# Bowen951209/raytracing-book

Measured on AMD Instinct MI355X. Metric: Msamples/sec (W×H×spp/s) on Book-2 final scene @1080p, 1/2/4/8 GPUs, higher is better.
Workload: dtype f32

## Files before the change

### include/rt/rt_debug.h

```cpp
#ifndef RT_DEBUG_H
#define RT_DEBUG_H

#include <stddef.h>

#ifdef __cplusplus
extern "C" {
#endif

int rt_debug_eval_builtin(int device, int fn, const float* x, const float* y, float* out, int n);

int rt_debug_threaded_bvh(const void* nodes, size_t nbytes, void* out, size_t out_cap, int* n_out);

int rt_debug_fast_tables(const void* bvh, size_t nbytes, const void* quads, size_t qbytes, const void* boxes,
                         size_t bbytes, int n_spheres, void* nodes_out, size_t nodes_cap, int* n_per_octant,
                         unsigned int* info_out, size_t info_cap, int* slots_out, int* n_slots);

int rt_debug_link_nodes(const void* bvh, size_t nbytes, void* out, size_t out_cap, int* n_f4);
int rt_debug_link_nodes_vbox(const void* bvh, size_t nbytes, const float* vbox, int n_box, void* out,
                             size_t out_cap, int* n_f4, int* n_nodes);
int rt_debug_collapse_links(const void* bvh, size_t nbytes, const float cam[28], int width, int height, int rebuild,
                            void* out, size_t out_cap, int* n_f4, unsigned char* drop, size_t drop_cap,
                            int* n_dropped);

int rt_debug_perlin_pack(const float* texels, int w, int h, void* out, size_t out_cap);
// ... 16 lines not shown

int rt_debug_device_count(void);

int rt_debug_ab_build(void);

enum {
    RT_OPTION_BOX_PRETEST = 1,
    RT_OPTION_FASTDIV = 2,
    RT_OPTION_SPH_LDS = 3,
    RT_OPTION_BIG_WG = 4,
    RT_OPTION_CHUNK_TARGET = 5,
    RT_OPTION_STAGED_CHUNK_TARGET = 6,
    RT_OPTION_STAGE_TILES = 7,
    RT_OPTION_SM_BATCH = 8,
    RT_OPTION_SM_FRAC = 9,
    RT_OPTION_WALK_FRAC = 10,
    RT_OPTION_WATCHDOG_MS = 11,
    RT_OPTION_CHUNK_WAIT_MS = 12,
    RT_OPTION_LDS_NODE_CAP = 13,
    RT_OPTION_COMPACT_BOXES = 14,
    RT_OPTION_SPINE = 15,
    RT_OPTION_TL_LEAF_LDS = 16,
    RT_OPTION_PERLIN_PACKED = 17,
    RT_OPTION_SPARSE_STAGE = 18,
    RT_OPTION_SPHERE_PAIRS = 19,
    RT_OPTION_LEAF_PREFETCH = 20,
    RT_OPTION_TL_SMALL_LDS = 21,
    RT_OPTION_SHADE_LDS = 22,
    RT_OPTION_BOX_VNODES = 23,
    RT_OPTION_ZERO_DIR_END = 24,
    RT_OPTION_COLLAPSE = 25,
    RT_OPTION_REBUILD = 26,
    RT_OPTION_TAIL_CHUNKS = 27,
    RT_OPTION_KERNEL_VARIANT = 100,
    RT_OPTION_DEBUG_FLAGS = 101
};
int rt_debug_set_option(struct rt_ctx* ctx, int option, int value);
int rt_debug_get_option(struct rt_ctx* ctx, int option, int* value);

int rt_debug_last_launch(struct rt_ctx* ctx, int* out, int n);

int rt_debug_walk_bvh(struct rt_ctx* ctx, void* out, size_t out_cap, size_t* nbytes);

int rt_debug_build_sah_bvh(const void* spheres, size_t sph_bytes, const void* quads, size_t quad_bytes,
                           const void* media, size_t med_bytes, const void* boxes, size_t box_bytes,
                           const void* bvh, size_t bvh_bytes, int order, const float eye[3],
                           float prim_cost, void* out, size_t out_cap, size_t* nbytes);

#ifdef __cplusplus
}
#endif

#endif
```

### raytracing-book_amd/csrc/rt_capi.hip

```cpp
#include <hip/hip_runtime.h>

#include <algorithm>
#include <chrono>
#include <climits>
#include <cmath>
#include <cstdio>
#include <cstdlib>
#include <cstring>
#include <functional>
#include <map>
#include <string>
#include <thread>
#include <vector>

#include <dlfcn.h>
#include <rccl/rccl.h>

#include "rt/rt.h"
#include "rt/rt_debug.h"
#include "rt/rt_types.h"
#include "rt_device.h"
#include "bvh_sah.h"

namespace {
// ... 88 lines not shown
    std::vector<float4> inner2;
    std::vector<uint2> leaves2;
    int depth = 0;
};

}

struct rt_ctx {
    std::vector<Device> devs;
    std::string err;
    std::vector<uint8_t> host_buf[6];
    bool uploaded[6] = {false, false, false, false, false, false};
    int tex_format[8] = {0}, tex_w[8] = {0}, tex_h[8] = {0};
    rt_camera_ubo cam{};
    bool have_cam = false;
    int max_depth = 5;
    float background[3] = {0, 0, 0};
    float sqrt_spp = 1.0f, recip_sqrt_spp = 1.0f;
    int width = 0, height = 0;
    int proc_rank = 0, proc_world = 1, stripe_rows = 16;
    int n_dnodes = 0;
    std::vector<rt_dnode> dnodes;
    int bvh_mode = RT_BVH_REFERENCE;
    int n_link_nodes = 0;
    std::vector<uint8_t> sah_bvh;
    std::vector<rt_dnode> walk_dn;
    std::vector<float4> walk_links;
    int n_walk_nodes = 0;
    bool walk_v = false;
    float walk_v_margin = -1.0f;
    bool walk_stale = true;
    std::vector<float4> boxc_host;
    bool box_vnodes = true;
    bool zero_dir_end = true;
    bool collapse = true;
    int rebuild = 2;
    bool walk_r = false;
    int walk_rmode = 0;
    std::vector<rt_dnode> rb_dn;
    int rb_mode = -1;
    bool walk_c = false;
    rt_camera_ubo walk_cam{};
    int walk_w = 0, walk_h = 0;
    int n_dropped = 0;
    int n_rebuilt = 0;
    int n_vnodes = 0;
    FastTables fast;
    std::vector<float4> links;
    int fast_gen = 0;
    bool spec_ok = false;
    int debug_flags = 0;
    bool uv_always = false;
    bool boxes_canon = false;
    bool fd_ok[6] = {true, true, true, true, true, true};
    bool fd_cam = true;
    bool boxes_cond = false;
    float scene_extent = -1.0f;
    bool validated = false;
    uint64_t last_ns = 0;
    int variant = 0;
    int variant_no_stats = -1;
    std::vector<int64_t> inj_hits;
    int64_t inj_walks = 0;
    int chunk_target = 16;
    int staged_chunk_target = 48;
    int tail_chunks = -1;
// ... 1710 lines not shown
    a.chunk_wait_ticks = c->chunk_wait_ticks;
    int32_t lc = 0;
    if (c->host_buf[RT_BIND_LIGHTS].size() >= 4) std::memcpy(&lc, c->host_buf[RT_BIND_LIGHTS].data(), 4);
    a.lights_count = lc;
    a.uv_always = c->uv_always;
    a.boxes_canon = c->boxes_canon ? 1 : 0;
    if (c->scene_extent < 0.0f) c->scene_extent = scene_extent(c);
    a.box_margin = (c->boxes_cond && c->box_pretest && c->scene_extent <= 0x1p60f)
                       ? std::max(c->scene_extent, 1.0f) * 0x1p-13f
                       : 0.0f;
    a.fastdiv = (c->fastdiv && c->fd_cam && c->fd_ok[RT_BIND_SPHERES] && c->fd_ok[RT_BIND_QUADS] &&
                 c->fd_ok[RT_BIND_BOXES])
                    ? 1
                    : 0;
    a.variant = c->variant;
    a.zero_dir_end = c->zero_dir_end ? 1 : 0;
    a.sm_batch = c->sm_batch;
    a.walk_frac = c->walk_frac ? c->walk_frac : walk_frac_for(c->n_link_nodes);
    const FastTables& F = c->fast;
    a.fast_ok = F.ok ? 1 : 0;
    a.n_f2inner = (int)(F.inner2.size() / 4);
    a.n_f2leaves = (int)F.leaves2.size();
    a.f2depth = F.depth;
    std::memcpy(a.finfo_base, F.base, sizeof(a.finfo_base));
    a.fm_n = F.fm_n;
    std::memcpy(a.fm_medium, F.fm_medium, sizeof(a.fm_medium));
    std::memcpy(a.fm_leaf, F.fm_leaf, sizeof(a.fm_leaf));
    std::memcpy(a.fm_track, F.fm_track, sizeof(a.fm_track));
    std::memcpy(a.fm_flags, F.fm_flags, sizeof(a.fm_flags));
    a.fl_n = F.fl_n;
    std::memcpy(a.fl_medium, F.fl_medium, sizeof(a.fl_medium));
    std::memcpy(a.fl_rank, F.fl_rank, sizeof(a.fl_rank));
    a.debug_flags = c->debug_flags;
    {
        const size_t nb = c->host_buf[RT_BIND_BOXES].size() / sizeof(rt_box);
        const bool all_cmp = c->compact_boxes && nb > 0 && c->n_boxc_ok == (int)nb;
        const bool use_v = c->box_vnodes && all_cmp && a.box_margin > 0.0f && (c->variant == 0 || c->variant == 39) &&
                           c->boxc_host.size() == nb * RT_BOXC_F4;
        const bool use_c = c->collapse && (c->variant == 0 || c->variant == 39) && c->have_cam;
        const bool cam_moved = use_c && (std::memcmp(&c->walk_cam, &c->cam, sizeof(rt_camera_ubo)) != 0 ||
                                         c->walk_w != c->width || c->walk_h != c->height);
        const bool use_r = c->rebuild > 0 && (c->variant == 0 || c->variant == 39);
        if (c->walk_stale || use_v != c->walk_v || (use_v && a.box_margin != c->walk_v_margin) ||
            use_c != c->walk_c || cam_moved || use_r != c->walk_r || c->rebuild != c->walk_rmode) {
            if (c->walk_stale) c->rb_mode = -1;
            if (use_r && c->rb_mode != c->rebuild) {
                c->rb_dn = rebuild_inner(c->walk_dn, c->rebuild);
                c->rb_mode = c->rebuild;
            }
            static const std::vector<rt_dnode> none;
            const std::vector<rt_dnode>& rb = use_r ? c->rb_dn : none;
            const std::vector<rt_dnode>& wdn = rb.empty() ? c->walk_dn : rb;
            std::vector<uint8_t> drop;
            if (use_c) {
                try {
                    if (!c->inj_hits.empty() && c->inj_hits.size() >= wdn.size()) {
                        std::vector<uint32_t> order{0u};
                        for (size_t q = 0; q < order.size() && order.size() <= wdn.size(); q++) {
                            const uint32_t k = order[q];
                            if ((wdn[k].meta & 0xF0000u) != 0 || k + 1 >= wdn.size()) continue;
                            order.push_back(k + 1);
                            order.push_back(wdn[k + 1].meta & 0xFFFFu);
                        }
                        std::vector<int64_t> H(wdn.size(), 0);
                        if (order.size() == wdn.size())
                            for (size_t q = 0; q < order.size(); q++)
// ... 931 lines not shown
        int r = d2h(c, d, tmp.data(), d.stats.ptr, sizeof(unsigned long long) * n);
        if (r) return r;
        for (int i = 0; i < n; i++) out[i] += tmp[i];
    }
    return RT_OK;
}

int rt_debug_ab_build(void) {
#ifdef RT_AB_KNOBS
    return 1;
#else
    return 0;
#endif
}

int rt_debug_set_option(rt_ctx* c, int option, int v) {
    if (!c) return RT_ERR_INVALID_ARG;
    auto bad = [&]() { return set_err(c, RT_ERR_INVALID_ARG, "option value out of range"); };
    switch (option) {
        case RT_OPTION_BOX_PRETEST: c->box_pretest = v != 0; break;
        case RT_OPTION_FASTDIV: c->fastdiv = v != 0; break;
        case RT_OPTION_SPH_LDS: c->sph_lds = v != 0; break;
        case RT_OPTION_BIG_WG: c->big_wg = v != 0; break;
        case RT_OPTION_COMPACT_BOXES: c->compact_boxes = v != 0; break;
        case RT_OPTION_SPINE: c->spine = v != 0; break;
        case RT_OPTION_TL_LEAF_LDS: c->tl_leaf_lds = v != 0; break;
        case RT_OPTION_PERLIN_PACKED: c->perlin_pk = v != 0; break;
        case RT_OPTION_SPARSE_STAGE: c->sparse_stage = v != 0; break;
        case RT_OPTION_SPHERE_PAIRS: if (v < 0 || v > 2) return bad(); c->sphere_pairs = v; break;
        case RT_OPTION_LEAF_PREFETCH: c->leaf_prefetch = v != 0; break;
        case RT_OPTION_TL_SMALL_LDS: c->tl_small_lds = v != 0; break;
        case RT_OPTION_SHADE_LDS: c->shade_lds = v != 0; break;
        case RT_OPTION_BOX_VNODES: c->box_vnodes = v != 0; break;
        case RT_OPTION_ZERO_DIR_END: c->zero_dir_end = v != 0; break;
        case RT_OPTION_COLLAPSE: c->collapse = v != 0; break;
        case RT_OPTION_REBUILD: if (v < 0 || v > 2) return bad(); c->rebuild = v; break;
        case RT_OPTION_CHUNK_TARGET: if (v < 0) return bad(); c->chunk_target = v; break;
        case RT_OPTION_STAGED_CHUNK_TARGET: if (v < 1) return bad(); c->staged_chunk_target = v; break;
        case RT_OPTION_STAGE_TILES: if (v < 0) return bad(); c->stage_tiles = v; break;
        case RT_OPTION_SM_BATCH: if (v < 1 || v > 64) return bad(); c->sm_batch = v; break;
        case RT_OPTION_SM_FRAC: if (v < 0 || v > 64) return bad(); c->sm_frac = v; break;
        case RT_OPTION_WALK_FRAC: if (v < 0 || v > 64) return bad(); c->walk_frac = v; break;
        case RT_OPTION_WATCHDOG_MS: if (v < 0) return bad(); c->watchdog_ticks = (unsigned long long)v * 100000ull; break;
        case RT_OPTION_CHUNK_WAIT_MS: if (v < 0) return bad(); c->chunk_wait_ticks = (unsigned long long)v * 100000ull; break;
        case RT_OPTION_LDS_NODE_CAP: if (v < 0) return bad(); c->lds_node_cap = v; break;
        case RT_OPTION_TAIL_CHUNKS: if (v < -1 || v > RT_MAX_FRAMES_PER_LAUNCH) return bad(); c->tail_chunks = v; break;
#ifdef RT_AB_KNOBS
        case RT_OPTION_KERNEL_VARIANT:
            if (!(v == 0 || v == 30 || v == 31 || v == 37 || v == 38 || v == 39 || v == 61 || v == 69)) return bad();
            c->variant = v;
            break;
        case RT_OPTION_DEBUG_FLAGS: c->debug_flags = v; break;
#endif
        default: return set_err(c, RT_ERR_INVALID_ARG, "unknown option (A/B options need librtamd_ab.so)");
    }
    return RT_OK;
}

int rt_debug_get_option(rt_ctx* c, int option, int* v) {
    if (!c || !v) return RT_ERR_INVALID_ARG;
    switch (option) {
        case RT_OPTION_BOX_PRETEST: *v = c->box_pretest; break;
        case RT_OPTION_FASTDIV: *v = c->fastdiv; break;
        case RT_OPTION_SPH_LDS: *v = c->sph_lds; break;
        case RT_OPTION_BIG_WG: *v = c->big_wg; break;
        case RT_OPTION_COMPACT_BOXES: *v = c->compact_boxes; break;
        case RT_OPTION_SPINE: *v = c->spine; break;
        case RT_OPTION_TL_LEAF_LDS: *v = c->tl_leaf_lds; break;
        case RT_OPTION_PERLIN_PACKED: *v = c->perlin_pk; break;
        case RT_OPTION_SPARSE_STAGE: *v = c->sparse_stage; break;
        case RT_OPTION_SPHERE_PAIRS: *v = c->sphere_pairs; break;
        case RT_OPTION_LEAF_PREFETCH: *v = c->leaf_prefetch; break;
        case RT_OPTION_TL_SMALL_LDS: *v = c->tl_small_lds; break;
        case RT_OPTION_SHADE_LDS: *v = c->shade_lds; break;
        case RT_OPTION_BOX_VNODES: *v = c->box_vnodes; break;
        case RT_OPTION_ZERO_DIR_END: *v = c->zero_dir_end; break;
        case RT_OPTION_COLLAPSE: *v = c->collapse; break;
        case RT_OPTION_REBUILD: *v = c->rebuild; break;
        case RT_OPTION_CHUNK_TARGET: *v = c->chunk_target; break;
        case RT_OPTION_STAGED_CHUNK_TARGET: *v = c->staged_chunk_target; break;
        case RT_OPTION_STAGE_TILES: *v = c->stage_tiles; break;
        case RT_OPTION_SM_BATCH: *v = c->sm_batch; break;
        case RT_OPTION_SM_FRAC: *v = c->sm_frac; break;
        case RT_OPTION_WALK_FRAC: *v = c->walk_frac; break;
        case RT_OPTION_WATCHDOG_MS: *v = (int)std::min<unsigned long long>(INT_MAX, c->watchdog_ticks / 100000ull); break;
        case RT_OPTION_CHUNK_WAIT_MS: *v = (int)std::min<unsigned long long>(INT_MAX, c->chunk_wait_ticks / 100000ull); break;
        case RT_OPTION_LDS_NODE_CAP: *v = c->lds_node_cap; break;
        case RT_OPTION_TAIL_CHUNKS: *v = c->tail_chunks; break;
#ifdef RT_AB_KNOBS
        case RT_OPTION_KERNEL_VARIANT: *v = c->variant; break;
        case RT_OPTION_DEBUG_FLAGS: *v = c->debug_flags; break;
#endif
        default: return set_err(c, RT_ERR_INVALID_ARG, "unknown option (A/B options need librtamd_ab.so)");
    }
    return RT_OK;
}

int rt_set_bvh_mode(rt_ctx* c, int mode) {
    if (!c) return RT_ERR_INVALID_ARG;
    if (mode != RT_BVH_REFERENCE && mode != RT_BVH_SAH) return set_err(c, RT_ERR_INVALID_ARG, "bad BVH mode");
    if (mode != c->bvh_mode) {
        c->bvh_mode = mode;
        c->validated = false;
    }
    return RT_OK;
}

int rt_debug_walk_bvh(rt_ctx* c, void* out, size_t out_cap, size_t* nbytes) {
// ... 53 lines not shown
```

### raytracing-book_amd/csrc/rt_device.h

```cpp
#pragma once

#include <hip/hip_runtime.h>
#include <stdint.h>

#include "rt/rt_types.h"

#define RT_MAX_FRAMES_PER_LAUNCH 512
#define RT_NODE_END 0xFFFFu
#define RT_DFACE_F4 3
#define RT_DBOX_F4 23
#define RT_BOXC_F4 3
#define RT_LDS_ACC_BYTES (512 * 16)
#define RT_LDS_DYN_BYTES (80 * 1024 - RT_LDS_ACC_BYTES)
#define RT_LDS_BIG_BYTES (160 * 1024)
#define RT_LDS_BIG_STATS_BYTES (150 * 1024)
#define RT_CENSUS_WORDS 5
#define RT_STATS_N 128
#define RT_LDS_NODE_BYTES (64 * 1024)

struct rt_dnode {
    float xmin, xmax, ymin, ymax, zmin, zmax;
    uint32_t meta;
    uint32_t prims;
};
// ... 61 lines not shown
    int perlin_slot;
    int perlin_lds;
    int perlin_packed;
    const float4* perlin_pk;
    int n_media;
    int media_sph;
    int media_lds;
    int sph_lds;
    int n_sph_lds;
    int n_box_lds;
    int sph_mat_lds;
    int box_mat_lds;
    int tex_lds;
    int tex_lds_off[8];
    int block;
    int acc_lds;
    const uint32_t* finfo;
    int fast_ok;
    int finfo_base[8];
    int fm_n;
    int fm_medium[4], fm_leaf[4], fm_track[4], fm_flags[4];
    int fl_n;
    int fl_medium[2], fl_rank[2];
    const float4* f2inner;
    const uint2* f2leaves;
    int n_f2inner, n_f2leaves, f2depth;
    const float4* lnodes;
    int n_lnode_f4;
    int lds_node_f4;
    int leaf_lds;
    int lds_end_f4;
    int box_cmp_lds;
    int box_all_cmp;
    int sph_pairs;
    int spine_len;
    uint32_t spine_start;
    float spine_lo[3], spine_hi[3];
    unsigned long long watchdog_ticks;
    unsigned long long chunk_wait_ticks;
    float rand_factors[RT_MAX_FRAMES_PER_LAUNCH];
};

enum { RT_LI_SHAPE = 0, RT_LI_BLOCK, RT_LI_FASTDIV, RT_LI_PRETEST, RT_LI_LDS, RT_LI_LDS_NODES, RT_LI_COMPACT,
       RT_LI_STAGED, RT_LI_CHUNKS, RT_LI_SPINE, RT_LI_SPARSE, RT_LI_SPAIR, RT_LI_LEAF_PF, RT_LI_SHADE_LDS, RT_LI_WALK_FRAC, RT_LI_BVH_MODE, RT_LI_VNODES, RT_LI_COLLAPSED, RT_LI_REBUILT, RT_LI_N = 20 };

#ifdef RT_AB_KNOBS
#define RT_FAST_STACK 16
enum { RT_AB_SHAPE_FAST_LDS = 0, RT_AB_SHAPE_FAST_GLOBAL, RT_AB_SHAPE_LINK_PIXEL, RT_AB_SHAPE_META_LDS,
       RT_AB_SHAPE_META_GLOBAL };
int rt_launch_render_ab(int shape, rt_kernel_args& a, const rt_kernel_args* d, size_t lds, bool stats, void* stream);
#endif
int rt_resident_waves(void);
int rt_launch_render(rt_kernel_args& a, rt_kernel_args* dargs, void* stream, int* info, void* moments = nullptr);
int rt_launch_fold_moments(const rt_kernel_args& a, void* moments, void* stream);
int rt_launch_tile_sums(const void* image, const void* moments, int width, int local_rows, void* out, void* stream);
__host__ __device__ inline void rt_gathered_row(int y, int world, int stripe_rows, int* k, int* lr) {
    const int s = y / stripe_rows;
    *k = s % world;
    *lr = (s / world) * stripe_rows + y % stripe_rows;
}
int rt_launch_deinterleave(const void* gathered, void* out, int width, int height, int world, int stripe_rows,
                           int padded_rows, void* stream);
int rt_launch_eval_builtin(int fn, const float* dx, const float* dy, float* dout, int n, void* stream);
```

### raytracing-book_amd/csrc/rt_kernel.hip

```cpp
#include "rt_kernel_common.h"

namespace {

#define RT_SM_FRESH 0
#define RT_SM_TRACE 1
#define RT_SM_HIT 2
#define RT_SM_BEGIN 4
struct UnitGeo {
    int chunk, tile, tx0, ly0, wt, ht, f0, f1;
    uint32_t total;
};
__device__ __forceinline__ UnitGeo unit_geo(const KP& P, int u, int n_tiles, int tiles_x) {
    UnitGeo g;
    g.chunk = u / n_tiles;
    g.tile = u - g.chunk * n_tiles;
    g.tx0 = (g.tile % tiles_x) * 8;
    g.ly0 = (g.tile / tiles_x) * 8;
    g.wt = min(8, P.width - g.tx0);
    g.ht = min(8, P.local_rows - g.ly0);
    const int c_main = P.n_chunks - P.tail_chunks;
    if (g.chunk < c_main) {
        g.f0 = g.chunk * P.chunk_frames;
        g.f1 = min(P.n_frames - P.tail_chunks, g.f0 + P.chunk_frames);
    } else {
// ... 219 lines not shown
        RT_ST_PART(ST_BEGIN_CYC)
        __builtin_amdgcn_s_setprio(1);
        for (;;) {
            unsigned long long th = STATS ? clock64() : 0;
            const unsigned long long tr = __ballot(status == RT_SM_TRACE);
            const int n_hit = __popcll(__ballot(status == RT_SM_HIT));
            if (STATS && tr) st_pred(st, status == RT_SM_FRESH, ST_RET_IT, ST_RET_LN);
            if (tr == 0 || n_hit >= batch || n_hit * 64 >= P.sm_frac * (n_hit + __popcll(tr))) break;
            const bool lane_exact = (inv.x == -INFINITY) || (inv.y == -INFINITY) || (inv.z == -INFINITY);
            const bool wave_exact = __ballot(status == RT_SM_TRACE && lane_exact) != 0;
            if (STATS) st_add(st, ST_RHEAD_CYC, clock64() - th);
            if (status == RT_SM_TRACE) {
                if (STATS) st_lanes(st, ST_ROUND_IT, ST_ROUND_LN);
                unsigned long long t0 = STATS ? clock64() : 0;
                if (P.walk_frac >= 64) {
                    nx = wave_exact ? link_walk<true, STATS, TL>(ns, nx, S.o, inv, 0.001f, tmax, st)
                                    : link_walk<false, STATS, TL>(ns, nx, S.o, inv, 0.001f, tmax, st);
                } else {
                    const int needw = (__popcll(__ballot(1)) * P.walk_frac + 63) >> 6;
                    nx = wave_exact ? link_walk_part<true, STATS, TL>(ns, nx, S.o, inv, 0.001f, tmax, needw, st)
                                    : link_walk_part<false, STATS, TL, (BOXC || (RT_BL_SPAIR && (OPT & RT_OPT_SPAIR) != 0)) && STD>(ns, nx, S.o, inv, 0.001f, tmax,
                                                                                    needw, st);
                }
                if (STATS) st_add(st, ST_NODE_CYC, clock64() - t0);
                if ((int)nx >= 0) {
                } else if (nx == RT_LINK_END) {
                    status = RT_SM_HIT;
                } else {
                    unsigned long long t1 = STATS ? clock64() : 0;
                    if (STATS) st_lanes(st, ST_LEAF_IT, ST_LEAF_LN);
                    uint2 lf;
                    if (gleaf) lf = ldg_u2(gleaves + (nx & 0x7FFFFFFFu));
                    else lf = leaves[nx & 0x7FFFFFFFu];
                    leaf_prims_t<STATS, FD, BOXC, (OPT & RT_OPT_SPAIR) != 0, STD>(P, lf.x << 16, lf.y, S.o, S.d, inv, a,
                                                                             S.time, 0.001f, tmax, S.rf,
                                                  fx, fy, h, has, st);
                    if (STATS) {
                        const unsigned long long t2 = clock64();
                        st_add(st, ST_LEAF_CYC, t2 - t1);
                        if (P.census) census_leaf(P, gwave, lf.x, t1, t2, __popcll(tr), st);
                    }
                    nx = lf.x >> 8;
                    if (nx == RT_LINK_NEXT_END) status = RT_SM_HIT;
                }
            }
        }
        __builtin_amdgcn_s_setprio(0);
        RT_ST_PART(ST_ROUNDS_CYC)
        if (status == RT_SM_HIT) {
            unsigned long long ts = STATS ? clock64() : 0;
            if (STATS) st_lanes(st, ST_SHADE_IT, ST_SHADE_LN);
            v3 cur3;
            h.t = tmax;
            bool done = after_trace<BOXC, STATS, STD>(P, S, h, has, fx, fy, cur3, st);
            if (!done && S.depth >= P.max_depth) {
                cur3 = mk3s(0.0f);
                done = true;
            } else if (!done && P.zero_dir_end && S.d.x == 0.0f && S.d.y == 0.0f && S.d.z == 0.0f) {
                cur3 = mul3(S.acc, mk3(P.background[0], P.background[1], P.background[2]));
                done = true;
            }
            if (done) {
                const float4 c4 = make_float4(cur3.x, cur3.y, cur3.z, 0.0f);
                if (staged) {
                    if (sparse) {
                        const bool nz = (__float_as_uint(cur3.x) | __float_as_uint(cur3.y) | __float_as_uint(cur3.z)) != 0u;
                        P.sflags[dst] = nz ? 1 : 0;
// ... 181 lines not shown
    a.leaf_pf = (a.leaf_pf && a.box_all_cmp && a.sph_lds >= 0 && a.box_cmp_lds > a.sph_lds &&
                 (a.n_media == 0 || a.media_lds >= 0)) ? 1 : 0;
    a.acc_lds = (int)(staged / 16);
    const size_t lds = staged + (pool ? 0 : RT_LDS_ACC_BYTES);
    if (info) {
        info[RT_LI_SHAPE] = (int)shape;
        info[RT_LI_BLOCK] = (shape == LINK_LDS || shape == LINK_TL) ? a.block : 512;
        info[RT_LI_FASTDIV] = a.fastdiv;
        info[RT_LI_PRETEST] = a.box_margin > 0.0f;
        info[RT_LI_LDS] = (int)lds;
        info[RT_LI_LDS_NODES] = (shape == LINK_LDS || shape == LINK_TL) ? a.lds_node_f4 / 2 : 0;
        info[RT_LI_COMPACT] = a.box_all_cmp + 2 * (a.box_cmp_lds >= 0);
        info[RT_LI_STAGED] = a.samples != nullptr;
        info[RT_LI_CHUNKS] = a.n_chunks;
        info[RT_LI_SPINE] = pool ? a.spine_len : 0;
        info[RT_LI_SPARSE] = a.samples && a.sflags ? 1 : 0;
        info[RT_LI_SPAIR] = (pool && shape == LINK_LDS && a.sph_lds >= 0 &&
                             ((a.sph_pairs && !a.box_all_cmp) || (a.sph_pairs == 2 && a.fastdiv))) ? 1 : 0;
        info[RT_LI_LEAF_PF] = (pool && (shape == LINK_LDS || shape == LINK_TL)) ? a.leaf_pf : 0;
        info[RT_LI_WALK_FRAC] = a.walk_frac;
        info[RT_LI_SHADE_LDS] = (a.sph_mat_lds >= 0) + 2 * (a.box_mat_lds >= 0) + 4 * (a.tex_lds >= 0);
    }
    if (hipMemcpyAsync(dargs, &a, sizeof(a), hipMemcpyHostToDevice, st) != hipSuccess) return -1;
    const rt_kernel_args* d = (const rt_kernel_args*)dargs;
    const int n_tiles = ((a.width + 7) / 8) * ((a.local_rows + 7) / 8);
    if (hipMemsetAsync(a.tile_counter, 0, sizeof(int), st) != hipSuccess) return -1;
    if (a.n_chunks > 1 && !a.samples &&
        hipMemsetAsync(a.tile_done, 0, sizeof(unsigned) * (size_t)n_tiles, st) != hipSuccess)
        return -1;

    constexpr int SM = RT_OPT_POOL | RT_OPT_SM | RT_OPT_STREAM;
#ifdef RT_AB_KNOBS
#define RT_KERNEL(BLOCK, OPT)                                                                            \
    (stats ? launch_persistent(render_persistent<4, true, BLOCK, OPT>, BLOCK, lds, a, d, st)                \
           : launch_persistent(render_persistent<4, false, BLOCK, OPT>, BLOCK, lds, a, d, st))
#else
#define RT_KERNEL(BLOCK, OPT) launch_persistent(render_persistent<4, false, BLOCK, OPT>, BLOCK, lds, a, d, st)
#endif
    int rc = -1;
    const bool std_cfg = a.samples && a.sflags && a.media_sph &&
                         (a.n_sph_lds == 0 || (a.sph_lds >= 0 && a.sph_mat_lds >= 0)) &&
                         (a.n_media == 0 || a.media_lds >= 0) && (a.n_box_lds == 0 || a.box_cmp_lds >= 0) &&
                         (!a.box_all_cmp || (a.leaf_pf && a.box_mat_lds >= 0)) && a.tex_lds >= 0;
#define RT_LINK4(BLOCK, OPT)                                                                                 \
    (a.fastdiv ? (a.box_all_cmp ? (std_cfg ? RT_KERNEL(BLOCK, (OPT) | RT_OPT_FD | RT_OPT_BOXC | RT_OPT_STD)            \
                                           : RT_KERNEL(BLOCK, (OPT) | RT_OPT_FD | RT_OPT_BOXC))                         \
                                : (std_cfg ? RT_KERNEL(BLOCK, (OPT) | RT_OPT_FD | RT_OPT_STD)                            \
                                           : RT_KERNEL(BLOCK, (OPT) | RT_OPT_FD)))                                      \
               : (a.box_all_cmp ? RT_KERNEL(BLOCK, (OPT) | RT_OPT_BOXC) : RT_KERNEL(BLOCK, (OPT))))
#define RT_LINK4S(BLOCK, OPT)                                                                                 \
    ((a.sph_pairs == 2 && a.box_all_cmp && a.fastdiv) ? RT_KERNEL(BLOCK, (OPT) | RT_OPT_FD | RT_OPT_BOXC | RT_OPT_SPAIR) : \
    (a.sph_pairs && !a.box_all_cmp)                                                                          \
         ? (a.fastdiv ? (std_cfg ? RT_KERNEL(BLOCK, (OPT) | RT_OPT_FD | RT_OPT_SPAIR | RT_OPT_STD)                      \
                                 : RT_KERNEL(BLOCK, (OPT) | RT_OPT_FD | RT_OPT_SPAIR))                                \
                      : RT_KERNEL(BLOCK, (OPT) | RT_OPT_SPAIR))                                                       \
         : RT_LINK4(BLOCK, OPT))
    switch (shape) {
        case LINK_LDS:
            if (!pool) {
#ifdef RT_AB_KNOBS
                rc = rt_launch_render_ab(RT_AB_SHAPE_LINK_PIXEL, a, d, lds, stats, st);
#endif
            } else if (a.block == 1024) {
                rc = RT_LINK4S(1024, SM);
            } else {
                rc = RT_LINK4S(512, SM);
            }
            break;
        case LINK_TL: rc = RT_LINK4(1024, SM | RT_OPT_TL); break;
#ifdef RT_AB_KNOBS
        case FAST_LDS: rc = rt_launch_render_ab(RT_AB_SHAPE_FAST_LDS, a, d, lds, stats, st); break;
        case FAST_GLOBAL: rc = rt_launch_render_ab(RT_AB_SHAPE_FAST_GLOBAL, a, d, lds, stats, st); break;
        case META_LDS: rc = rt_launch_render_ab(RT_AB_SHAPE_META_LDS, a, d, lds, stats, st); break;
        case META_GLOBAL: rc = rt_launch_render_ab(RT_AB_SHAPE_META_GLOBAL, a, d, lds, stats, st); break;
#endif
        default: break;
    }
#undef RT_KERNEL
// ... 28 lines not shown
```

### raytracing-book_amd/csrc/rt_kernel_common.h

```cpp
#pragma once

#include <hip/hip_runtime.h>

#include <algorithm>
#include <cstdio>
#include <cstdlib>

#include "rt/rt_glsl.h"
#include "rt_device.h"


namespace {

typedef rt_kernel_args KP;

#ifndef RT_BL_SPAIR
#define RT_BL_SPAIR 1
#endif
#define RT_OPT_POOL 1
#define RT_OPT_SM 2
#define RT_OPT_FD 4
#define RT_OPT_STREAM 8
#define RT_OPT_TL 16
#define RT_OPT_BOXC 32
#define RT_OPT_SPAIR 64
#define RT_OPT_STD 128

extern __shared__ float4 rt_dyn_lds[];

__device__ __forceinline__ v3 f3(float4 v) { return mk3(v.x, v.y, v.z); }

typedef float f4v __attribute__((ext_vector_type(4)));
typedef __attribute__((address_space(1))) const f4v g_f4v;
typedef __attribute__((address_space(1))) const float g_f;
typedef __attribute__((address_space(3))) const float lds_f;
__device__ __forceinline__ float4 ldg(const float4* p) {
    const f4v v = *(const g_f4v*)p;
    return make_float4(v.x, v.y, v.z, v.w);
}
__device__ __forceinline__ int ldg_i(const int* p) { return *(__attribute__((address_space(1))) const int*)p; }
typedef __attribute__((address_space(4))) const f4v c_f4v;
__device__ __forceinline__ float4 ldc(const float4* p) {
    const f4v v = *(const c_f4v*)p;
    return make_float4(v.x, v.y, v.z, v.w);
}
__device__ __forceinline__ int ldc_i(const int* p) { return *(__attribute__((address_space(4))) const int*)p; }
typedef unsigned u2v __attribute__((ext_vector_type(2)));
__device__ __forceinline__ uint2 ldg_u2(const uint2* p) {
    const u2v v = *(__attribute__((address_space(1))) const u2v*)p;
    return make_uint2(v.x, v.y);
}

enum {
    ST_TOTAL = 0, ST_START_CYC, ST_START_IT, ST_START_LN, ST_NODE_CYC, ST_NODE_IT, ST_NODE_LN, ST_LEAF_CYC,
    ST_LEAF_IT, ST_LEAF_LN, ST_SPH_LN, ST_QUAD_LN, ST_BOX_LN, ST_MED_LN, ST_SHADE_CYC, ST_SHADE_IT, ST_SHADE_LN,
    ST_SPH_IT, ST_QUAD_IT, ST_BOX_IT, ST_MED_IT,
    ST_FAST_TRACES, ST_FAST_EXACT, ST_FAST_WHY, ST_FAST_STEPS = ST_FAST_WHY + 9, ST_FAST_TESTS,
    ST_FAST_PRE_CYC, ST_FAST_POST_CYC, ST_FAST_EXACT_CYC,
// ... 177 lines not shown
            ti[k] = (pl.w - g_dot(n, o)) / denom;
            if (!(fabsf(denom) < 1e-8f) && (tmin <= ti[k] && ti[k] <= tmax)) cand |= 1u << k;
        }
#pragma unroll
        for (int k = 0; k < 3; k++) {
            const int i = h + k;
            if ((cand >> k) & 1u) {
                float al, be;
                if (ti[k] <= tmax && face_interior(ldg(fb + 6 + 2 * i), ldg(fb + 7 + 2 * i), o, d, ti[k], al, be, fd)) {
                    tmax = ti[k];
                    t = ti[k];
                    face = i;
                    alpha = al;
                    beta = be;
                    has = true;
                }
            }
        }
    }
    return has;
}

template <int I>
__device__ __forceinline__ void boxc_face(float mnx, float mny, float mnz, float mxx, float mxz, float DX, float DY,
                                          float DZ, float4& A, float4& B) {
    if (I == 0) { A = make_float4(mnx, mny, DX, 0.0f); B = make_float4(0.0f, DY, DX * DY, __int_as_float(0)); }
    if (I == 1) { A = make_float4(mny, mxz, 0.0f, -DZ); B = make_float4(DY, 0.0f, DZ * DY, __int_as_float(2)); }
    if (I == 2) { A = make_float4(mxx, mny, -DX, 0.0f); B = make_float4(0.0f, DY, -(DX * DY), __int_as_float(0)); }
    if (I == 3) { A = make_float4(mny, mnz, 0.0f, DZ); B = make_float4(DY, 0.0f, -(DZ * DY), __int_as_float(2)); }
    if (I == 4) { A = make_float4(mnx, mxz, DX, 0.0f); B = make_float4(0.0f, -DZ, -(DX * DZ), __int_as_float(1)); }
    if (I == 5) { A = make_float4(mnx, mnz, DX, 0.0f); B = make_float4(0.0f, DZ, DX * DZ, __int_as_float(1)); }
}
__device__ __forceinline__ bool box_test_compact(float4 c0, float4 c1, float4 c2, v3 o, v3 d, float tmin, float tmax,
                                                 float& t, int& face, float& alpha, float& beta, bool fd = false) {
    const float mnx = c0.x, mny = c0.y, mnz = c0.z, mxx = c0.w, mxy = c1.x, mxz = c1.y;
    const float sz = c1.z, sx = c1.w, sy = c2.x;
    bool has = false;
#define RT_BOXC_FACE(I, S, Q, DK, OK)                                                           \
    {                                                                                                      \
        const float s_ = (S), den = s_ * (DK);                                                             \
        float ti;                                                                                          \
        if (fd) {                                                                                          \
            ti = div_nr(s_ * (Q) - s_ * (OK), den, rcp_nr(den));                                           \
        } else {                                                                                           \
            ti = (s_ * (Q) - s_ * (OK)) / den;                                                             \
        }                                                                                                  \
        if (!(fabsf(den) < 1e-8f) && (tmin <= ti && ti <= tmax)) {                                         \
            float4 A, B;                                                                                   \
            boxc_face<I>(mnx, mny, mnz, mxx, mxz, mxx - mnx, mxy - mny, mxz - mnz, A, B);                  \
            float al, be;                                                                                  \
            if (face_interior(A, B, o, d, ti, al, be, fd)) {                                               \
                tmax = ti;                                                                                 \
                t = ti;                                                                                    \
                face = I;                                                                                  \
                alpha = al;                                                                                \
                beta = be;                                                                                 \
                has = true;                                                                                \
            }                                                                                              \
        }                                                                                                  \
    }
    RT_BOXC_FACE(0, sz, mxz, d.z, o.z)
    RT_BOXC_FACE(1, sx, mxx, d.x, o.x)
    RT_BOXC_FACE(2, -sz, mnz, d.z, o.z)
    RT_BOXC_FACE(3, -sx, mnx, d.x, o.x)
    RT_BOXC_FACE(4, sy, mxy, d.y, o.y)
    RT_BOXC_FACE(5, -sy, mny, d.y, o.y)
#undef RT_BOXC_FACE
    return has;
}

__device__ __noinline__ bool boundary_t(const KP& P, int idx, int type, v3 o, v3 d, float a, float time, float tmin,
                                           float tmax, float& t) {
    float al, be;
    int face;
    if (type == RT_MODEL_SPHERE)
        return sphere_t(reinterpret_cast<const float4*>(P.spheres + idx), time, o, d, a, tmin, tmax, t);
    if (type == RT_MODEL_QUAD) return quad_test(P.dquads + RT_DFACE_F4 * idx, o, d, tmin, tmax, t, al, be);
    if (type == RT_MODEL_BOX) return box_test(P.dboxes + RT_DBOX_F4 * idx, o, d, tmin, tmax, t, face, al, be);
    return false;
}

__device__ __forceinline__ bool sphere_bounds(float4 A, float4 B, v3 o, v3 d, float a, float time, float& t1,
                                              float& t2, bool fd = false) {
    {
        v3 center = add3(f3(A), scale3(f3(B), time));
        v3 oc = sub3(o, center);
        float half_b = g_dot(oc, d);
        float c = g_dot(oc, oc) - B.w * B.w;
        float disc = half_b * half_b - a * c;
        float sq = sqrtf(disc);
        fd = fd && __ballot(!(a >= 0x1p-60f)) == 0;
        const float ra = fd ? rcp_nr(a) : 0.0f;
        float r_lo = fd ? div_nr(-half_b - sq, a, ra) : (-half_b - sq) / a;
        float r_hi = fd ? div_nr(-half_b + sq, a, ra) : (-half_b + sq) / a;
        const bool lo_in = -RT_INFINITY < r_lo && r_lo < RT_INFINITY;
        const bool hi_in = -RT_INFINITY < r_hi && r_hi < RT_INFINITY;
        t1 = lo_in ? r_lo : r_hi;
        const float lo2 = t1 + 0.0001f;
        const bool lo_2 = lo2 < r_lo && r_lo < RT_INFINITY;
        const bool hi_2 = lo2 < r_hi && r_hi < RT_INFINITY;
// ... 89 lines not shown
    float r;
    asm("v_max_f32 %0, %1, %2" : "=v"(r) : "v"(a), "v"(b));
    return r;
}
__device__ __forceinline__ float v_min3(float a, float b, float c) {
    float r;
    asm("v_min3_f32 %0, %1, %2, %3" : "=v"(r) : "v"(a), "v"(b), "v"(c));
    return r;
}
__device__ __forceinline__ float v_max3(float a, float b, float c) {
    float r;
    asm("v_max3_f32 %0, %1, %2, %3" : "=v"(r) : "v"(a), "v"(b), "v"(c));
    return r;
}
__device__ __forceinline__ bool aabb_fast(float4 n0, float4 n1, v3 o, v3 inv, float tmin, float tmax) {
    float t0x = (n0.x - o.x) * inv.x, t1x = (n0.y - o.x) * inv.x;
    float t0y = (n0.z - o.y) * inv.y, t1y = (n0.w - o.y) * inv.y;
    float t0z = (n1.x - o.z) * inv.z, t1z = (n1.y - o.z) * inv.z;
    float lo = v_max(v_max3(tmin, v_min(t0x, t1x), v_min(t0y, t1y)), v_min(t0z, t1z));
    float hi = v_min(v_min3(tmax, v_max(t0x, t1x), v_max(t0y, t1y)), v_max(t0z, t1z));
    return !(hi <= lo);
}

typedef float f2v __attribute__((ext_vector_type(2)));
__device__ __forceinline__ bool aabb_pk(float4 n0, float4 n1, v3 o, v3 inv, float tmin, float tmax) {
    const f2v tx = (f2v{n0.x, n0.y} - f2v{o.x, o.x}) * f2v{inv.x, inv.x};
    const f2v ty = (f2v{n0.z, n0.w} - f2v{o.y, o.y}) * f2v{inv.y, inv.y};
    const f2v tz = (f2v{n1.x, n1.y} - f2v{o.z, o.z}) * f2v{inv.z, inv.z};
    float lo = v_max(v_max3(tmin, v_min(tx.x, tx.y), v_min(ty.x, ty.y)), v_min(tz.x, tz.y));
    float hi = v_min(v_min3(tmax, v_max(tx.x, tx.y), v_max(ty.x, ty.y)), v_max(tz.x, tz.y));
    return !(hi <= lo);
}

template <bool STATS, bool FD, bool BOXC = false, bool SPAIR = false, bool STD = false>
__device__ __forceinline__ void leaf_prims_t(const KP& P, uint32_t meta, uint32_t prims, v3 o, v3 d, v3 inv, float a,
                                             float time, float tmin, float& tmax, float& rf, float px, float py, Hit& h,
                                             bool& has, unsigned long long* st) {
    constexpr bool fd = FD;
    if (SPAIR && !STATS && (STD || P.sph_lds >= 0) && ((meta >> 16) & 0xFFu) == (RT_MODEL_SPHERE | (RT_MODEL_SPHERE << 4))) {
        const int i0 = (int)(prims & 0xFFFFu), i1 = (int)(prims >> 16);
        const float4* r0 = rt_dyn_lds + P.sph_lds + 2 * i0;
        const float4* r1 = rt_dyn_lds + P.sph_lds + 2 * i1;
        const float4 A0 = r0[0], B0 = r0[1], A1 = r1[0], B1 = r1[1];
        float lo0, hi0, lo1, hi1;
        const bool ok0 = sphere_roots(A0, B0, time, o, d, a, lo0, hi0, fd);
        const bool ok1 = sphere_roots(A1, B1, time, o, d, a, lo1, hi1, fd);
#pragma unroll
        for (int k = 0; k < 2; k++) {
            const bool ok = k ? ok1 : ok0;
            const int ix = k ? i1 : i0;
            float root = k ? lo1 : lo0;
            bool hit = ok && tmin < root && root < tmax;
            if (ok && !hit) {
                root = k ? hi1 : hi0;
                hit = tmin < root && root < tmax;
            }
            if (hit) {
                h.uv_kind_idx = (1 << 16) | ix;
                h.uv_a = root;
                has = true;
                tmax = root;
                h.t = root;
                h.tif = RT_MODEL_SPHERE | (ix << 16);
            }
        }
        return;
    }
// ... 44 lines not shown
                hit = sphere_t(reinterpret_cast<const float4*>(P.spheres + ix), time, o, d, a, tmin, tmax, t, fd,
                               fd ? rcp_nr(a) : 0.0f);
            }
            if (hit) { h.uv_kind_idx = (1 << 16) | ix; h.uv_a = t; }
            if (STATS) st_add(st, ST_SPH_CYC, clock64() - c0);
        } else if (ty == RT_MODEL_QUAD) {
            hit = quad_test(P.dquads + RT_DFACE_F4 * ix, o, d, tmin, tmax, t, al, be, fd);
            if (hit) { h.uv_kind_idx = 2 << 16; h.uv_a = al; h.uv_b = be; }
            if (STATS) st_add(st, ST_QUAD_CYC, clock64() - c0);
        } else if (ty == RT_MODEL_BOX) {
            float4 r0, r1, r2;
            if (pf) {
                r0 = q0;
                r1 = q1;
                r2 = q2;
            } else if (STD || P.box_cmp_lds >= 0) {
                const float4* cr = rt_dyn_lds + P.box_cmp_lds + RT_BOXC_F4 * ix;
                r0 = cr[0];
                r1 = cr[1];
                r2 = cr[2];
            } else {
                const float4* cr = P.dboxc + RT_BOXC_F4 * ix;
                r0 = ldg(cr);
                r1 = ldg(cr + 1);
                r2 = ldg(cr + 2);
            }
            bool maybe = true;
            if (P.box_margin > 0.0f && (BOXC || fin) && !pretested) {
                const float m = P.box_margin;
                maybe = aabb_pk(make_float4(r0.x - m, r0.w + m, r0.y - m, r1.x + m),
                                make_float4(r0.z - m, r1.y + m, 0.0f, 0.0f), o, inv, tmin, tmax);
            }
            if (maybe) {
                if constexpr (BOXC)
                    hit = box_test_compact(r0, r1, r2, o, d, tmin, tmax, t, face, al, be, fd);
                else
                    hit = box_test(P.dboxes + RT_DBOX_F4 * ix, o, d, tmin, tmax, t, face, al, be, fd);
            }
            if (hit) { h.uv_kind_idx = 2 << 16; h.uv_a = al; h.uv_b = be; }
            if (STATS) st_add(st, ST_BOX_CYC, clock64() - c0);
        } else if (ty == RT_MODEL_CONSTANT_MEDIUM) {
            hit = pf ? medium_test_rec<FD, STD>(P, q0, q1, q2, o, d, a, time, tmin, tmax, rf, px, py, t)
                     : medium_test<FD, STD>(P, ix, o, d, a, time, tmin, tmax, rf, px, py, t);
            if (STATS) st_add(st, ST_MED_CYC, clock64() - c0);
        }
        if (hit) {
            has = true;
            tmax = t;
            h.t = t; h.tif = ty | (face << 4) | (ix << 16);
        }
    }
}


typedef __attribute__((address_space(3))) const f4v lds_f4;
struct NodeSrc {
    const char* base;
    const char* gnodes;
    uint32_t lim;
    unsigned* hits;
};
__device__ __forceinline__ void count_node_hit(unsigned* hits, uint32_t nx, bool hit) {
    const uint32_t n0 = __builtin_amdgcn_readfirstlane(nx);
    const unsigned long long hm = __ballot(hit && nx == n0);
    if (hm && first_active_lane()) atomicAdd(&hits[n0 >> 5], (unsigned)__popcll(hm));
    if (hit && nx != n0) atomicAdd(&hits[nx >> 5], 1u);
}
template <bool STATS, bool TL>
// ... 752 lines not shown
```

### raytracing-book_amd/rtamd/render.py

```python
import ctypes
import time

import numpy as np

from . import _lib
from ._lib import RTError, c_float_p
from .scene import Scene, spp_uniforms

MASK64 = (1 << 64) - 1


def frame_rand_factors(seed, start, n):
    out = np.empty(n, dtype=np.float32)
    for k in range(n):
        z = (seed + (start + k + 1) * 0x9E3779B97F4A7C15) & MASK64
        z = ((z ^ (z >> 30)) * 0xBF58476D1CE4E5B9) & MASK64
        z = ((z ^ (z >> 27)) * 0x94D049BB133111EB) & MASK64
        z ^= z >> 31
        out[k] = np.float32(z >> 40) / np.float32(16777216.0)
    return out


def comm_unique_id(lib=None):
    L = lib or _lib.amd()
# ... 22 lines not shown
    return out.raw[:n.value]


def local_rows(height, rank, world, stripe_rows):
    n_stripes = (height + stripe_rows - 1) // stripe_rows
    return sum(min(stripe_rows, height - s * stripe_rows) for s in range(rank, n_stripes, world))


def padded_local_rows(height, world, stripe_rows):
    n_stripes = (height + stripe_rows - 1) // stripe_rows
    return ((n_stripes + world - 1) // world) * stripe_rows


def stripe_rows_of(height, rank, world, stripe_rows):
    n_stripes = (height + stripe_rows - 1) // stripe_rows
    rows = []
    for s in range(rank, n_stripes, world):
        rows.extend(range(s * stripe_rows, min(height, (s + 1) * stripe_rows)))
    return np.array(rows, dtype=np.int64)


def deinterleave(gathered, height, world, stripe_rows):
    W = gathered.shape[2]
    out = np.zeros((height, W, 4), dtype=gathered.dtype)
    for k in range(world):
        rows = stripe_rows_of(height, k, world, stripe_rows)
        out[rows] = gathered[k, :len(rows)]
    return out


OPTIONS = {"box_pretest": 1, "fastdiv": 2, "sph_lds": 3, "big_wg": 4, "chunk_target": 5,
           "staged_chunk_target": 6, "stage_tiles": 7, "sm_batch": 8, "sm_frac": 9, "walk_frac": 10,
           "watchdog_ms": 11, "chunk_wait_ms": 12, "lds_node_cap": 13, "compact_boxes": 14, "spine": 15,
           "tl_leaf_lds": 16, "perlin_packed": 17, "sparse_stage": 18, "sphere_pairs": 19, "leaf_prefetch": 20, "tl_small_lds": 21, "shade_lds": 22, "box_vnodes": 23, "zero_dir_end": 24, "collapse": 25, "rebuild": 26, "tail_chunks": 27, "kernel_variant": 100, "debug_flags": 101}
LAUNCH_FIELDS = ("shape", "block", "fastdiv", "pretest", "lds_bytes", "lds_nodes", "box_records", "staged",
                 "chunks", "spine", "sparse", "sphere_pairs", "leaf_prefetch", "shade_lds", "walk_frac", "bvh_mode",
                 "box_vnodes", "collapsed", "rebuilt")
BVH_MODES = {"reference": 0, "sah": 1}
TILE_SUM_DTYPE = np.dtype([("m2y", "<f4"), ("y", "<f4"), ("bad", "<u4"), ("pixels", "<u4")])


def noise_from_tile_sums(tiles, frames, lib=None):
    L = lib or _lib.amd()
    t = np.ascontiguousarray(tiles, dtype=TILE_SUM_DTYPE)
    s = _lib.RtNoiseStats()
    rc = L.rt_noise_from_tile_sums(t.ctypes.data_as(ctypes.POINTER(_lib.RtTileSum)), int(t.size), int(frames),
                                   ctypes.byref(s))
    if rc != 0:
        raise RTError(rc, "rt_noise_from_tile_sums: frames >= 2 required")
    return s.as_dict()
SHAPES = {0: "fast-lds", 1: "fast-global", 2: "link-lds", 3: "meta-lds", 4: "meta-global", 5: "link-two-level"}


class RenderContext:

    def __init__(self, devices=(0,), rank=0, world=1, stripe_rows=16, options=None, ab=False, lib=None):
        L = _lib.amd_at(lib) if lib else (_lib.amd_ab() if ab else _lib.amd())
        self._L = L
        devs = (ctypes.c_int * len(devices))(*devices)
        h = ctypes.c_void_p()
        rc = L.rt_create(len(devices), devs, ctypes.byref(h))
        if rc != 0:
            raise RTError(rc, L.rt_last_error(None).decode())
        self._h = h
        self.devices = tuple(devices)
        self.rank, self.world, self.stripe_rows = rank, world, stripe_rows
        if world > 1 or stripe_rows != 16:
            self._check(L.rt_set_partition(h, rank, world, stripe_rows))
        self.width = self.height = 0
        self.max_depth = 5
# ... 278 lines not shown
```

Baseline: 7416.

## Add quotient-based box face interior test deferring divisions to final hit

Adds a new compact box intersection path that tests whether a face hit lies inside the face by comparing numerators against the denominator by sign and magnitude, instead of dividing to get alpha and beta for every candidate face. The slab distances for each axis pair now share one reciprocal, and the divisions for alpha and beta run only once, for the winning face. If any lane in the wave sees tiny or degenerate numerators, the whole wave falls back to the original routine through a ballot. The path is on by default for the standard compact-box, fast-divide, non-two-level, non-stats kernel, and it adds a new kernel template instantiation.

```diff
diff --git a/include/rt/rt_debug.h b/include/rt/rt_debug.h
--- a/include/rt/rt_debug.h
+++ b/include/rt/rt_debug.h
@@ -72,6 +72,7 @@
     RT_OPTION_COLLAPSE = 25,
     RT_OPTION_REBUILD = 26,
     RT_OPTION_TAIL_CHUNKS = 27,
+    RT_OPTION_BOX_INTERIOR = 28,
     RT_OPTION_KERNEL_VARIANT = 100,
     RT_OPTION_DEBUG_FLAGS = 101
 };
diff --git a/raytracing-book_amd/csrc/rt_capi.hip b/raytracing-book_amd/csrc/rt_capi.hip
--- a/raytracing-book_amd/csrc/rt_capi.hip
+++ b/raytracing-book_amd/csrc/rt_capi.hip
@@ -144,6 +144,7 @@
     bool walk_stale = true;
     std::vector<float4> boxc_host;
     bool box_vnodes = true;
+    bool box_interior = true;
     bool zero_dir_end = true;
     bool collapse = true;
     int rebuild = 2;
@@ -1920,6 +1921,7 @@
     std::memcpy(a.fl_medium, F.fl_medium, sizeof(a.fl_medium));
     std::memcpy(a.fl_rank, F.fl_rank, sizeof(a.fl_rank));
     a.debug_flags = c->debug_flags;
+    a.box_interior = c->box_interior ? 1 : 0;
     {
         const size_t nb = c->host_buf[RT_BIND_BOXES].size() / sizeof(rt_box);
         const bool all_cmp = c->compact_boxes && nb > 0 && c->n_boxc_ok == (int)nb;
@@ -2917,6 +2919,7 @@
         case RT_OPTION_TL_SMALL_LDS: c->tl_small_lds = v != 0; break;
         case RT_OPTION_SHADE_LDS: c->shade_lds = v != 0; break;
         case RT_OPTION_BOX_VNODES: c->box_vnodes = v != 0; break;
+        case RT_OPTION_BOX_INTERIOR: c->box_interior = v != 0; break;
         case RT_OPTION_ZERO_DIR_END: c->zero_dir_end = v != 0; break;
         case RT_OPTION_COLLAPSE: c->collapse = v != 0; break;
         case RT_OPTION_REBUILD: if (v < 0 || v > 2) return bad(); c->rebuild = v; break;
@@ -2959,6 +2962,7 @@
         case RT_OPTION_TL_SMALL_LDS: *v = c->tl_small_lds; break;
         case RT_OPTION_SHADE_LDS: *v = c->shade_lds; break;
         case RT_OPTION_BOX_VNODES: *v = c->box_vnodes; break;
+        case RT_OPTION_BOX_INTERIOR: *v = c->box_interior; break;
         case RT_OPTION_ZERO_DIR_END: *v = c->zero_dir_end; break;
         case RT_OPTION_COLLAPSE: *v = c->collapse; break;
         case RT_OPTION_REBUILD: *v = c->rebuild; break;
diff --git a/raytracing-book_amd/csrc/rt_device.h b/raytracing-book_amd/csrc/rt_device.h
--- a/raytracing-book_amd/csrc/rt_device.h
+++ b/raytracing-book_amd/csrc/rt_device.h
@@ -117,6 +117,7 @@
     int lds_end_f4;
     int box_cmp_lds;
     int box_all_cmp;
+    int box_interior;
     int sph_pairs;
     int spine_len;
     uint32_t spine_start;
@@ -127,7 +128,7 @@
 };
 
 enum { RT_LI_SHAPE = 0, RT_LI_BLOCK, RT_LI_FASTDIV, RT_LI_PRETEST, RT_LI_LDS, RT_LI_LDS_NODES, RT_LI_COMPACT,
-       RT_LI_STAGED, RT_LI_CHUNKS, RT_LI_SPINE, RT_LI_SPARSE, RT_LI_SPAIR, RT_LI_LEAF_PF, RT_LI_SHADE_LDS, RT_LI_WALK_FRAC, RT_LI_BVH_MODE, RT_LI_VNODES, RT_LI_COLLAPSED, RT_LI_REBUILT, RT_LI_N = 20 };
+       RT_LI_STAGED, RT_LI_CHUNKS, RT_LI_SPINE, RT_LI_SPARSE, RT_LI_SPAIR, RT_LI_LEAF_PF, RT_LI_SHADE_LDS, RT_LI_WALK_FRAC, RT_LI_BVH_MODE, RT_LI_VNODES, RT_LI_COLLAPSED, RT_LI_REBUILT, RT_LI_BOXQ, RT_LI_N = 20 };
 
 #ifdef RT_AB_KNOBS
 #define RT_FAST_STACK 16
diff --git a/raytracing-book_amd/csrc/rt_kernel.hip b/raytracing-book_amd/csrc/rt_kernel.hip
--- a/raytracing-book_amd/csrc/rt_kernel.hip
+++ b/raytracing-book_amd/csrc/rt_kernel.hip
@@ -275,7 +275,7 @@
                     uint2 lf;
                     if (gleaf) lf = ldg_u2(gleaves + (nx & 0x7FFFFFFFu));
                     else lf = leaves[nx & 0x7FFFFFFFu];
-                    leaf_prims_t<STATS, FD, BOXC, (OPT & RT_OPT_SPAIR) != 0, STD>(P, lf.x << 16, lf.y, S.o, S.d, inv, a,
+                    leaf_prims_t<STATS, FD, BOXC, (OPT & RT_OPT_SPAIR) != 0, STD, (OPT & RT_OPT_BOXQ) != 0>(P, lf.x << 16, lf.y, S.o, S.d, inv, a,
                                                                              S.time, 0.001f, tmax, S.rf,
                                                   fx, fy, h, has, st);
                     if (STATS) {
@@ -523,7 +523,7 @@
     constexpr int SM = RT_OPT_POOL | RT_OPT_SM | RT_OPT_STREAM;
 #ifdef RT_AB_KNOBS
 #define RT_KERNEL(BLOCK, OPT)                                                                            \
-    (stats ? launch_persistent(render_persistent<4, true, BLOCK, OPT>, BLOCK, lds, a, d, st)                \
+    (stats ? launch_persistent(render_persistent<4, true, BLOCK, (OPT) & ~RT_OPT_BOXQ>, BLOCK, lds, a, d, st)  \
            : launch_persistent(render_persistent<4, false, BLOCK, OPT>, BLOCK, lds, a, d, st))
 #else
 #define RT_KERNEL(BLOCK, OPT) launch_persistent(render_persistent<4, false, BLOCK, OPT>, BLOCK, lds, a, d, st)
@@ -533,8 +533,13 @@
                          (a.n_sph_lds == 0 || (a.sph_lds >= 0 && a.sph_mat_lds >= 0)) &&
                          (a.n_media == 0 || a.media_lds >= 0) && (a.n_box_lds == 0 || a.box_cmp_lds >= 0) &&
                          (!a.box_all_cmp || (a.leaf_pf && a.box_mat_lds >= 0)) && a.tex_lds >= 0;
+    if (info)
+        info[RT_LI_BOXQ] = (pool && !stats && a.box_interior && a.fastdiv && a.box_all_cmp && std_cfg &&
+                            shape == LINK_LDS && a.sph_pairs != 2) ? 1 : 0;
 #define RT_LINK4(BLOCK, OPT)                                                                                 \
-    (a.fastdiv ? (a.box_all_cmp ? (std_cfg ? RT_KERNEL(BLOCK, (OPT) | RT_OPT_FD | RT_OPT_BOXC | RT_OPT_STD)            \
+    (a.fastdiv ? (a.box_all_cmp ? (std_cfg ? (a.box_interior             \
+                                                  ? RT_KERNEL(BLOCK, (OPT) | RT_OPT_FD | RT_OPT_BOXC | RT_OPT_STD | (((OPT) & RT_OPT_TL) ? 0 : RT_OPT_BOXQ)) \
+                                                  : RT_KERNEL(BLOCK, (OPT) | RT_OPT_FD | RT_OPT_BOXC | RT_OPT_STD))      \
                                            : RT_KERNEL(BLOCK, (OPT) | RT_OPT_FD | RT_OPT_BOXC))                         \
                                 : (std_cfg ? RT_KERNEL(BLOCK, (OPT) | RT_OPT_FD | RT_OPT_STD)                            \
                                            : RT_KERNEL(BLOCK, (OPT) | RT_OPT_FD)))                                      \
diff --git a/raytracing-book_amd/csrc/rt_kernel_common.h b/raytracing-book_amd/csrc/rt_kernel_common.h
--- a/raytracing-book_amd/csrc/rt_kernel_common.h
+++ b/raytracing-book_amd/csrc/rt_kernel_common.h
@@ -24,6 +24,7 @@
 #define RT_OPT_TL 16
 #define RT_OPT_BOXC 32
 #define RT_OPT_SPAIR 64
+#define RT_OPT_BOXQ 256
 #define RT_OPT_STD 128
 
 extern __shared__ float4 rt_dyn_lds[];
@@ -267,7 +268,8 @@
     if (I == 5) { A = make_float4(mnx, mnz, DX, 0.0f); B = make_float4(0.0f, DZ, DX * DZ, __int_as_float(1)); }
 }
 __device__ __forceinline__ bool box_test_compact(float4 c0, float4 c1, float4 c2, v3 o, v3 d, float tmin, float tmax,
-                                                 float& t, int& face, float& alpha, float& beta, bool fd = false) {
+                                                 float& t, int& face, float& alpha, float& beta, bool fd = false,
+                                                 bool abl = false) {
     const float mnx = c0.x, mny = c0.y, mnz = c0.z, mxx = c0.w, mxy = c1.x, mxz = c1.y;
     const float sz = c1.z, sx = c1.w, sy = c2.x;
     bool has = false;
@@ -283,8 +285,8 @@
         if (!(fabsf(den) < 1e-8f) && (tmin <= ti && ti <= tmax)) {                                         \
             float4 A, B;                                                                                   \
             boxc_face<I>(mnx, mny, mnz, mxx, mxz, mxx - mnx, mxy - mny, mxz - mnz, A, B);                  \
-            float al, be;                                                                                  \
-            if (face_interior(A, B, o, d, ti, al, be, fd)) {                                               \
+            float al = 0.5f, be = 0.5f;                                                                    \
+            if (abl || face_interior(A, B, o, d, ti, al, be, fd)) {                                        \
                 tmax = ti;                                                                                 \
                 t = ti;                                                                                    \
                 face = I;                                                                                  \
@@ -301,6 +303,74 @@
     RT_BOXC_FACE(4, sy, mxy, d.y, o.y)
     RT_BOXC_FACE(5, -sy, mny, d.y, o.y)
 #undef RT_BOXC_FACE
+    return has;
+}
+
+__device__ __forceinline__ bool unit_quotients(float na, float nb, float delta) {
+    const int dl = __float_as_int(delta);
+    return ((__float_as_int(na) ^ dl) | (__float_as_int(nb) ^ dl)) >= 0 && fmaxf(fabsf(na), fabsf(nb)) <= fabsf(delta);
+}
+
+__device__ __forceinline__ bool box_test_compact_q(float4 c0, float4 c1, float4 c2, v3 o, v3 d, float tmin,
+                                                   const float tmax0, float& t, int& face, float& alpha, float& beta,
+                                                   bool abl = false) {
+    const float mnx = c0.x, mny = c0.y, mnz = c0.z, mxx = c0.w, mxy = c1.x, mxz = c1.y;
+    const float sz = c1.z, sx = c1.w, sy = c2.x;
+    float tmax = tmax0, tq = 0.0f, qa = 0.0f, qb = 0.0f, qd = 1.0f;
+    int fq = -1;
+    bool odd = false;
+#define RT_BOXQ_AXIS(S, DK, OK, QA, QB, TA, TB, OKD)                                                       \
+    float TA, TB;                                                                                          \
+    bool OKD;                                                                                              \
+    {                                                                                                      \
+        const float s_ = (S), den = s_ * (DK), so = s_ * (OK), r = rcp_nr(den);                            \
+        TA = div_nr(s_ * (QA) - so, den, r);                                                               \
+        TB = div_nr(s_ * (QB) - so, den, r);                                                               \
+        OKD = !(fabsf(den) < 1e-8f);                                                                       \
+    }
+#define RT_BOXQ_FACE(I, TI, OKD)                                                                           \
+    if ((OKD) && (tmin <= (TI) && (TI) <= tmax)) {                                                         \
+        float4 A, B;                                                                                       \
+        boxc_face<I>(mnx, mny, mnz, mxx, mxz, mxx - mnx, mxy - mny, mxz - mnz, A, B);                      \
+        const int cs = __float_as_int(B.w);                                                                \
+        const float oa = (cs == 2) ? o.y : o.x, da = (cs == 2) ? d.y : d.x;                                \
+        const float ob = (cs == 0) ? o.y : o.z, db = (cs == 0) ? d.y : d.z;                                \
+        const float pa = (oa + da * (TI)) - A.x;                                                           \
+        const float pb = (ob + db * (TI)) - A.y;                                                           \
+             \
+                              \
+        const float na = ((I) == 1 || (I) == 3) ? -(pb * B.x) : pa * B.y;                                  \
+        const float nb = ((I) == 1 || (I) == 3) ? -(pa * A.w) : pb * A.z;                                  \
+        odd = odd || !(fabsf(na) >= 0x1p-100f && fabsf(nb) >= 0x1p-100f);                                  \
+        if (abl || unit_quotients(na, nb, B.z)) {                                                          \
+            tmax = (TI);                                                                                   \
+            tq = (TI);                                                                                     \
+            fq = I;                                                                                        \
+            qa = na;                                                                                       \
+            qb = nb;                                                                                       \
+            qd = B.z;                                                                                      \
+        }                                                                                                  \
+    }
+    RT_BOXQ_AXIS(sz, d.z, o.z, mxz, mnz, t0, t2, okz)
+    RT_BOXQ_AXIS(sx, d.x, o.x, mxx, mnx, t1, t3, okx)
+    RT_BOXQ_FACE(0, t0, okz)
+    RT_BOXQ_FACE(1, t1, okx)
+    RT_BOXQ_FACE(2, t2, okz)
+    RT_BOXQ_FACE(3, t3, okx)
+    RT_BOXQ_AXIS(sy, d.y, o.y, mxy, mny, t4, t5, oky)
+    RT_BOXQ_FACE(4, t4, oky)
+    RT_BOXQ_FACE(5, t5, oky)
+#undef RT_BOXQ_AXIS
+#undef RT_BOXQ_FACE
+    if (!abl && __ballot(odd) != 0) return box_test_compact(c0, c1, c2, o, d, tmin, tmax0, t, face, alpha, beta, true);
+    const bool has = fq >= 0;
+    if (has) {
+        const float r = rcp_nr(qd);
+        t = tq;
+        face = fq;
+        alpha = abl ? 0.5f : div_nr(qa, qd, r);
+        beta = abl ? 0.5f : div_nr(qb, qd, r);
+    }
     return has;
 }
 
@@ -456,7 +526,7 @@
     return !(hi <= lo);
 }
 
-template <bool STATS, bool FD, bool BOXC = false, bool SPAIR = false, bool STD = false>
+template <bool STATS, bool FD, bool BOXC = false, bool SPAIR = false, bool STD = false, bool BOXQ = false>
 __device__ __forceinline__ void leaf_prims_t(const KP& P, uint32_t meta, uint32_t prims, v3 o, v3 d, v3 inv, float a,
                                              float time, float tmin, float& tmax, float& rf, float px, float py, Hit& h,
                                              bool& has, unsigned long long* st) {
@@ -567,8 +637,15 @@
                                 make_float4(r0.z - m, r1.y + m, 0.0f, 0.0f), o, inv, tmin, tmax);
             }
             if (maybe) {
-                if constexpr (BOXC)
-                    hit = box_test_compact(r0, r1, r2, o, d, tmin, tmax, t, face, al, be, fd);
+#ifdef RT_AB_KNOBS
+                const bool abl = (P.debug_flags & 8) != 0;
+#else
+                constexpr bool abl = false;
+#endif
+                if constexpr (BOXC && BOXQ && FD && STD && !STATS)
+                    hit = box_test_compact_q(r0, r1, r2, o, d, tmin, tmax, t, face, al, be, abl);
+                else if constexpr (BOXC)
+                    hit = box_test_compact(r0, r1, r2, o, d, tmin, tmax, t, face, al, be, fd, abl);
                 else
                     hit = box_test(P.dboxes + RT_DBOX_F4 * ix, o, d, tmin, tmax, t, face, al, be, fd);
             }
diff --git a/raytracing-book_amd/rtamd/render.py b/raytracing-book_amd/rtamd/render.py
--- a/raytracing-book_amd/rtamd/render.py
+++ b/raytracing-book_amd/rtamd/render.py
@@ -78,10 +78,10 @@
 OPTIONS = {"box_pretest": 1, "fastdiv": 2, "sph_lds": 3, "big_wg": 4, "chunk_target": 5,
            "staged_chunk_target": 6, "stage_tiles": 7, "sm_batch": 8, "sm_frac": 9, "walk_frac": 10,
            "watchdog_ms": 11, "chunk_wait_ms": 12, "lds_node_cap": 13, "compact_boxes": 14, "spine": 15,
-           "tl_leaf_lds": 16, "perlin_packed": 17, "sparse_stage": 18, "sphere_pairs": 19, "leaf_prefetch": 20, "tl_small_lds": 21, "shade_lds": 22, "box_vnodes": 23, "zero_dir_end": 24, "collapse": 25, "rebuild": 26, "tail_chunks": 27, "kernel_variant": 100, "debug_flags": 101}
+           "tl_leaf_lds": 16, "perlin_packed": 17, "sparse_stage": 18, "sphere_pairs": 19, "leaf_prefetch": 20, "tl_small_lds": 21, "shade_lds": 22, "box_vnodes": 23, "zero_dir_end": 24, "collapse": 25, "rebuild": 26, "tail_chunks": 27, "box_interior": 28, "kernel_variant": 100, "debug_flags": 101}
 LAUNCH_FIELDS = ("shape", "block", "fastdiv", "pretest", "lds_bytes", "lds_nodes", "box_records", "staged",
                  "chunks", "spine", "sparse", "sphere_pairs", "leaf_prefetch", "shade_lds", "walk_frac", "bvh_mode",
-                 "box_vnodes", "collapsed", "rebuilt")
+                 "box_vnodes", "collapsed", "rebuilt", "box_interior")
 BVH_MODES = {"reference": 0, "sah": 1}
 TILE_SUM_DTYPE = np.dtype([("m2y", "<f4"), ("y", "<f4"), ("bad", "<u4"), ("pixels", "<u4")])
 
```

Result: faster. 7647, median of 6 (+3.1%).
